# lyeemax/IS-VINS

Hardware: AMD Instinct MI355X
Metric: sliding-window solves/sec (11 KF, ~300 landmarks) (higher is better)
Workload: dtype f64; 1 GPU; 1024 independent synthetic sliding windows per GPU (N=11 KF, Nvo=5, L=300 landmarks, F~1070 reprojection factors each; BASELINE config 4 batch of config-2 windows), full backendOptimization(): NUM_ITERATIONS=10 dogleg iterations + update() + double2vector + MargForward/MargBackward on every window; windows_per_gpu=1024, windows_total=1024, frames=11, landmarks=300, factors_total=1095427

## Files before the change

is-vins_amd/csrc/isv_backend.hip:

```cpp
#include <hip/hip_runtime.h>
#include <atomic>
#include <chrono>
#include <cstdio>
#include <cstdlib>
#include <cstring>
#include <string>
#include <thread>
#include <sched.h>
#include <vector>
#include <algorithm>
#include "isv_device_types.h"
#include "isv_kernels.h"

#include "isv_batch_buffers.h"

extern "C" int isv_abi_version(void) { return ISV_ABI_VERSION; }

extern "C" const char *isv_backend_last_error(const isv_backend_t *h) { return h ? h->err.c_str() : "null handle"; }

extern "C" void isv_backend_destroy(isv_backend_t *h) {
    if (!h) return;
    (void)hipSetDevice(h->device);
    if (h->graph_exec) (void)hipGraphExecDestroy(h->graph_exec);
    if (h->seq && h->seq_free) h->seq_free(h->seq);
// ... 531 lines not shown
        for (int i = 0; i < ISV_MAX_TRACE; i++) out[3] += act[i];
    }
    return ISV_OK;
}

static uint64_t fnv1a(const void *p, size_t n) { uint64_t x = 1469598103934665603ull; for (size_t i = 0; i < n; i++) { x ^= ((const unsigned char *)p)[i]; x *= 1099511628211ull; } return x; }

extern "C" int isv_batch_optimize(isv_backend_t *h, int32_t sync) {
    if (!h || !h->resident) return ISV_ERR_INVALID_ARG;
    ENTER(h);
    DevBatch &d = h->d; hipStream_t st = h->stream;
    memset(h->last_counts, 0, sizeof(h->last_counts));
    const bool profile = (sync & 2) != 0 && !h->prof_ev.empty();
    static const bool use_graph = getenv("ISV_GRAPH") != nullptr;
    if (use_graph && !profile) {
        d.sw_global = 0; d.ctl_stage_lm = 0; d.dg_stage_ph = 0;
        const uint64_t key = fnv1a(&d, sizeof(d));
        HIPCHK(h, hipEventRecord(h->ev[0], st));
        if (!h->graph_exec || h->graph_key != key) {
            if (h->graph_exec) { (void)hipGraphExecDestroy(h->graph_exec); h->graph_exec = nullptr; }
            hipGraph_t g = nullptr;
            HIPCHK(h, hipStreamBeginCapture(st, hipStreamCaptureModeThreadLocal));
            int rcg = ISV_OK;
            if (hipMemsetAsync(d.act, 0, sizeof(int32_t) * ISV_MAX_TRACE, st) != hipSuccess) rcg = ISV_ERR_DEVICE;
            if (rcg == ISV_OK) rcg = restore_initial(h);
            if (rcg == ISV_OK) {
                hipLaunchKernelGGL(k_vector2double, dim3(d.B), dim3(64), 0, st, d);
                rcg = isv_solver_enqueue(h->d, h->hc, st, h->stream2, h->fj, h->last_counts, nullptr, h->err);
            }
            const hipError_t ec = hipStreamEndCapture(st, &g);
            if (rcg != ISV_OK || ec != hipSuccess) { if (g) (void)hipGraphDestroy(g); h->err = "hipGraph capture failed"; return rcg != ISV_OK ? rcg : ISV_ERR_DEVICE; }
// ... 249 lines not shown
```

is-vins_amd/csrc/isv_build_solve_sb.hip:

```cpp
#include <hip/hip_runtime.h>
#include "isv_kernels.h"
#include "isv_device_math.h"
#include "isv_chain.h"
#include "isv_lin_gram.h"
#include "isv_rank1.h"
#include "isv_dogleg.h"

#ifdef ISV_STAMP
#define STAMP(k) do { if (t == 0) { unsigned long long now_ = wall_clock64(); d.dbg[(size_t)w * 64 + (k) + (MODE == 1 ? 32 : 0)] += (double)(now_ - t_last); t_last = now_; } } while (0)
#else
#define STAMP(k) do {} while (0)
#endif
#define LS 512
__host__ __device__ inline int sb_nred(int N, int prior_H_sz) {
    int m = LS;
    if (prior_H_sz > m) m = prior_H_sz;
    if (36 * N > m) m = 36 * N;
    if (30 * N > m) m = 30 * N;
    return (m + 1) & ~1;
}
#define RCH 32

DEV int sbt(int I, int J, int N) { return (I == J ? I : N + J) * 36; }

// ... 1037 lines not shown
            __syncthreads();
            if ((int)threadIdx.x >= 64 * nwaves) return;
            rank1_body<NT, TPW, 64, 1, EX>(d);
        }
    }
    else build_solve_sb_body<BIG, NC, 1>(d, lds);
}
template <bool BIG, int NC, bool EX>
__global__ __launch_bounds__(LS, 2) void k_pose_dogleg(DevBatch d) {
    extern __shared__ __align__(16) double lds[];
    __shared__ double red[256];
    __shared__ int s_accept;
    build_solve_sb_body<BIG, NC, 2>(d, lds);
    __syncthreads();
    if (threadIdx.x >= 256) return;
    dogleg_body<EX>(d, blockIdx.x, threadIdx.x, red);
    __syncthreads();
    step_control_body<true, EX>(d, blockIdx.x, threadIdx.x, lds, red, s_accept);
}
template __global__ void k_pose_dogleg<false, 11, false>(DevBatch);
template __global__ void k_pose_dogleg<false, 0, false>(DevBatch);
template __global__ void k_pose_dogleg<false, 0, true>(DevBatch);
template __global__ void k_lin_gram_chain<false, false, 0, 0>(DevBatch);
template __global__ void k_lin_gram_chain<false, false, 11, 0>(DevBatch);
template __global__ void k_lin_gram_chain<false, true, 0, 0>(DevBatch);
template __global__ void k_lin_gram_chain<true, false, 0, 0>(DevBatch);
template __global__ void k_lin_gram_chain<true, true, 0, 0>(DevBatch);
template __global__ void k_lin_gram_chain<false, true, 0, 7>(DevBatch);
template __global__ void k_build_solve_sb<false, 0, 0>(DevBatch);
template __global__ void k_build_solve_sb<false, 11, 0>(DevBatch);
template __global__ void k_build_solve_sb<true, 0, 0>(DevBatch);
template __global__ void k_build_solve_sb<false, 0, 1>(DevBatch);
template __global__ void k_build_solve_sb<false, 11, 1>(DevBatch);
// ... 18 lines not shown
```

is-vins_amd/csrc/isv_device_types.h:

```cpp
#pragma once
#include <stdint.h>
#include "../../include/isvins_backend.h"

#define ISV_TILE 64
#define ISV_MAX_FRAMES 32
#define ISV_MARG_WS 1408
#define ISV_SPLIT_MAX_GROUPS 32
#ifndef ISV_SPLIT_MIN_PASSES
#define ISV_SPLIT_MIN_PASSES 4
#endif
#define ISV_FUSED_MAX_FACTORS 8192
#define ISV_IMU_IN 64
#define IMU_DP 0
#define IMU_DQ 3
#define IMU_DV 7
#define IMU_LBA 10
#define IMU_LBG 13
#define IMU_DT 16
#define IMU_DP_DBA 17
#define IMU_DP_DBG 26
#define IMU_DQ_DBG 35
#define IMU_DV_DBA 44
#define IMU_DV_DBG 53

// ... 82 lines not shown
    double *st_ws;
    int32_t split_cap, _pad4;
    double *cs_ws;
    double *r1_part;
    double *Tvis;
    int32_t force_retry, init_mode;
    int32_t prior_H_sz, tvis_sz, wd_ld, max_lm;
    int32_t marg_scratch_sz, lds_T;
    int32_t force_invalid, _pad2;
    double min_radius;
    int32_t *pg_rec;
    double *pg_pts;
    int32_t *pg_wstart;
    double *flm;
    int32_t fused_visual;
    int32_t bs_split, _pad3;
    int32_t ctl_stage_lm, dg_stage_ph;
    int32_t lg_lcap;
    int32_t Nr, est_ex;
    double *Wex;
    double *flmx;
    double *ex_part;
    double *strip_ex;
};
```

is-vins_amd/csrc/isv_dogleg.h:

```cpp
#pragma once
#include <hip/hip_runtime.h>
#include "isv_kernels.h"
#include "isv_device_math.h"
#include "isv_proj_factor.h"
#include "isv_prior_factor.h"
#include "isv_imu_factor.h"

template <int K>
DEV void block_sums(double (&v)[K], double *red , int t) {
#pragma unroll
    for (int k = 0; k < K; k++) {
#pragma unroll
        for (int off = 32; off > 0; off >>= 1) v[k] += __shfl_down(v[k], off, 64);
    }
    if ((t & 63) == 0) {
#pragma unroll
        for (int k = 0; k < K; k++) red[(t >> 6) * K + k] = v[k];
    }
    __syncthreads();
#pragma unroll
    for (int k = 0; k < K; k++) v[k] = ((red[k] + red[K + k]) + red[2 * K + k]) + red[3 * K + k];
    __syncthreads();
}

#ifdef ISV_STAMP
#define DSTAMP(k) do { if (t == (k >= 56 ? 64 : 0)) { unsigned long long now_ = wall_clock64(); d.dbg[(size_t)w * 64 + (k)] += (double)(now_ - (k >= 56 ? t1_last : t_last)); if (k >= 56) t1_last = now_; else t_last = now_; } } while (0)
#else
#define DSTAMP(k) do {} while (0)
#endif
template <bool EX>
DEV void backsub_landmark(const DevBatch &d, const int l, const int fw0, const double *zs, const double *us, const double mu) {
            const unsigned m0 = d.lm_meta[l];
            const int h = (int)(m0 & 255), k = (int)((m0 >> 8) & 255);
            const double *wv = d.W + (size_t)(fw0 + (int)(m0 >> 16) + l) * 6;
            const double sl = d.scale_l[l], E = d.lmE[l], gl = d.lmG[l], Dl = d.diag_l[l];
            double wz = 0, wu = 0;
            for (int o = 0; o < k; o += 2) {
                const int o1 = o + 1 < k ? o + 1 : o;
                const double2 a01 = *reinterpret_cast<const double2 *>(wv + 6 * o), a23 = *reinterpret_cast<const double2 *>(wv + 6 * o + 2),
                              a45 = *reinterpret_cast<const double2 *>(wv + 6 * o + 4);
                const double2 b01 = *reinterpret_cast<const double2 *>(wv + 6 * o1), b23 = *reinterpret_cast<const double2 *>(wv + 6 * o1 + 2),
                              b45 = *reinterpret_cast<const double2 *>(wv + 6 * o1 + 4);
                const double *z = zs + 15 * (h + o), *u = us + 15 * (h + o);
                wz += a01.x * z[0] + a01.y * z[1] + a23.x * z[2] + a23.y * z[3] + a45.x * z[4] + a45.y * z[5];
                wu += a01.x * u[0] + a01.y * u[1] + a23.x * u[2] + a23.y * u[3] + a45.x * u[4] + a45.y * u[5];
                if (o + 1 < k) {
                    const double *z1 = zs + 15 * (h + o + 1), *u1 = us + 15 * (h + o + 1);
                    wz += b01.x * z1[0] + b01.y * z1[1] + b23.x * z1[2] + b23.y * z1[3] + b45.x * z1[4] + b45.y * z1[5];
                    wu += b01.x * u1[0] + b01.y * u1[1] + b23.x * u1[2] + b23.y * u1[3] + b45.x * u1[4] + b45.y * u1[5];
                }
            }
            if (EX) {
                const double *we = d.Wex + (size_t)l * 6, *z = zs + 15 * d.Nr, *u = us + 15 * d.Nr;
                for (int c6 = 0; c6 < 6; c6++) { wz += we[c6] * z[c6]; wu += we[c6] * u[c6]; }
            }
            const double Es = sl * sl * E, Dl2 = Dl * Dl;
            const double yl = (sl * gl - sl * wz) / (Es + mu * Dl2);
            d.gn_l[l] = -Dl * yl;
            const double ul = sl * sl * gl / Dl2, cl = sl * sl / (Es + mu * Dl2);
            d.lm_aterm[l] = cl * wu * wu + 2.0 * ul * wu + E * ul * ul;
}

template <bool EX>
DEV void dogleg_body(DevBatch &d, const int w, const int t, double *red) {
    SolveState &st = d.st[w];
    if (st.termination != ISV_TERM_RUNNING) return;
    const int n = d.np, N = d.N, l0 = d.lm_off[w], l1 = d.lm_off[w + 1];
    const double *gp = d.grad_p + (size_t)w * n, *gnp = d.gn_p + (size_t)w * n;
    const double *Dp = d.diag_p + (size_t)w * n, *scp = d.scale_p + (size_t)w * n;
    double *dp = d.delta_p + (size_t)w * n;
    if (st.ls_fail) {
        if (t == 0) { st.step_valid = 0; st.iteration += 1; st.fresh = 0; }
        return;
    }
#ifdef ISV_STAMP
    unsigned long long t_last = wall_clock64(), t1_last = t_last;
#endif
    if (d.lds_T) {
        extern __shared__ __align__(16) double dynp[];
        double *const sPr = dynp + (size_t)(N - 1) * 48 + (size_t)d.n_prior_slots * 16;
        prior_stage_records(d, w, sPr + (size_t)d.n_prior_slots * 20, t, 256);
        double *const sPHw = sPr + prior_lds_bytes(d.n_prior_slots, false) / sizeof(double) + 992 + n;
// ... 3 lines not shown
#pragma unroll
            for (int u = 0; u < 4; u++) { const int i = i0 + 256 * u; v4[u] = PHg[i < d.prior_H_sz ? i : d.prior_H_sz - 1]; }
#pragma unroll
            for (int u = 0; u < 4; u++) { const int i = i0 + 256 * u; if (i < d.prior_H_sz) sPHw[i] = v4[u]; }
        }
    }
    double a = 0, b = 0, c = 0, e = 0;
    for (int i = t; i < n; i += 256) { a += gp[i] * gp[i]; b += gnp[i] * gnp[i]; c += gp[i] * gnp[i]; }
    if (st.fresh && !d.bs_split) {
        extern __shared__ __align__(16) double dyn0[];
        double *zs = dyn0, *us = dyn0 + n;
        for (int i = t; i < n; i += 256) { zs[i] = d.zp[(size_t)w * n + i]; us[i] = d.up[(size_t)w * n + i]; }
        __syncthreads();
        const double mu = st.mu;
        const int fw0 = d.f_off[w];
        for (int l = l0 + t; l < l1; l += 256) backsub_landmark<EX>(d, l, fw0, zs, us, mu);
    }
    for (int lq = l0 + t; lq < l1; lq += 4 * 256) {
        double gl4[4], nl4[4], at4[4];
#pragma unroll
        for (int u = 0; u < 4; u++) { const int l = lq + 256 * u < l1 ? lq + 256 * u : l1 - 1; gl4[u] = d.grad_l[l]; nl4[u] = d.gn_l[l]; at4[u] = d.lm_aterm[l]; }
#pragma unroll
        for (int u = 0; u < 4; u++) if (lq + 256 * u < l1) { a += gl4[u] * gl4[u]; b += nl4[u] * nl4[u]; c += gl4[u] * nl4[u]; e += at4[u]; }
    }
    DSTAMP(48);
    double sums4[4] = {a, b, c, e};
    block_sums<4>(sums4, red, t);
    const double g2 = sums4[0], gn2 = sums4[1], gdotgn = sums4[2], aterm = sums4[3];
    double alpha = st.alpha;
    if (st.fresh) alpha = g2 / (st.qT + aterm);
    const double radius = st.radius, gn_norm = sqrt(gn2), g_norm = sqrt(g2);
    double cg, cn, step_norm_scaled;
// ... 1 lines not shown
    if (gn_norm <= radius) { cg = 0; cn = 1; step_norm_scaled = gn_norm; }
    else if (g_norm * alpha >= radius) { cg = -(radius / g_norm); cn = 0; step_norm_scaled = radius; }
    else {
        const double b_dot_a = -alpha * gdotgn;
        const double a_sq = pow(alpha * g_norm, 2.0);
        const double bma_sq = a_sq - 2 * b_dot_a + pow(gn_norm, 2.0);
        const double cc = b_dot_a - a_sq;
        const double dd = sqrt(cc * cc + bma_sq * (pow(radius, 2.0) - a_sq));
        const double beta = (cc <= 0) ? (dd - cc) / bma_sq : (radius * radius - a_sq) / (dd + cc);
        cg = -alpha * (1.0 - beta); cn = beta; step_norm_scaled = 0; need_norm = true;
    }
    double sn = 0;
    for (int i = t; i < n; i += 256) {
        const double s = cg * gp[i] + cn * gnp[i];
        sn += s * s;
        dp[i] = s / Dp[i] * scp[i];
    }
    for (int lq = l0 + t; lq < l1; lq += 4 * 256) {
        double gl4[4], nl4[4], dg4[4], sc4[4], lam4[4];
#pragma unroll
        for (int u = 0; u < 4; u++) { const int l = lq + 256 * u < l1 ? lq + 256 * u : l1 - 1; gl4[u] = d.grad_l[l]; nl4[u] = d.gn_l[l]; dg4[u] = d.diag_l[l]; sc4[u] = d.scale_l[l]; lam4[u] = d.lam[l]; }
#pragma unroll
        for (int u = 0; u < 4; u++) if (lq + 256 * u < l1) {
            const int l = lq + 256 * u;
            const double s = cg * gl4[u] + cn * nl4[u];
            sn += s * s;
            const double dl = s / dg4[u] * sc4[u];
            d.delta_l[l] = dl;
            d.clam[l] = lam4[u] + dl;
        }
    }
    double sums1[1] = {sn};
    block_sums<1>(sums1, red, t);
    const double sn_tot = sums1[0];
    if (need_norm) step_norm_scaled = sqrt(sn_tot);
    __syncthreads();
    double dn = 0, xn = 0;
    for (int i = t; i < N; i += 256) {
        const double *x = d.pose + ((size_t)w * N + i) * 7, *sb = d.sb + ((size_t)w * N + i) * 9;
        double *xc = d.cpose + ((size_t)w * N + i) * 7, *sc = d.csb + ((size_t)w * N + i) * 9;
        double xp[7];
        pose_plus(x, dp + 15 * i, xp);
        for (int k = 0; k < 7; k++) { xc[k] = xp[k]; const double df = x[k] - xp[k]; dn += df * df; xn += x[k] * x[k]; }
        for (int k = 0; k < 9; k++) { const double v = sb[k] + dp[15 * i + 6 + k]; sc[k] = v; const double df = sb[k] - v; dn += df * df; xn += sb[k] * sb[k]; }
    }
    for (int lq = l0 + t; lq < l1; lq += 4 * 256) {
        double lam4[4], cl4[4];
#pragma unroll
        for (int u = 0; u < 4; u++) { const int l = lq + 256 * u < l1 ? lq + 256 * u : l1 - 1; lam4[u] = d.lam[l]; cl4[u] = d.clam[l]; }
#pragma unroll
        for (int u = 0; u < 4; u++) if (lq + 256 * u < l1) { const double df = lam4[u] - cl4[u]; dn += df * df; xn += lam4[u] * lam4[u]; }
    }
    DSTAMP(49);
    double sums2[2] = {dn, xn};
    block_sums<2>(sums2, red, t);
    const double dn_tot = sums2[0], xn_tot = sums2[1];
    if (t == 0) {
        st.alpha = alpha; st.dogleg_step_norm = step_norm_scaled;
        st.step_norm = sqrt(dn_tot); st.x_norm = sqrt(xn_tot);
        st.step_valid = 1; st.iteration += 1; st.fresh = 0;
    }
    if (!d.lds_T) return;
    extern __shared__ __align__(16) double dyn[];
    const int NIw = N - 1, slots = d.n_prior_slots;
    double *sImu = dyn;
    double *sMod = sImu + NIw * 16;
    double *sPm = sMod + NIw * 32;
    double *sPrior = sPm + (size_t)slots * 16;
    {
        double *sDpw = sPrior + prior_lds_bytes(slots, false) / sizeof(double) + 992;
        for (int i = t; i < n; i += 256) sDpw[i] = dp[i];
    }
    __syncthreads();
    DSTAMP(50);
#ifdef ISV_STAMP
    t1_last = wall_clock64();
#endif
    const int lane = t & 63, wv = t >> 6;
    double *const sRaw = sPrior, *const sW = sPrior + (size_t)slots * 10;
    const PriorRecs PR = prior_recs_at(d, sPrior + (size_t)slots * 20);
    const int n_rp = d.n_rp[w];
    double *const sHb = sPrior + prior_lds_bytes(slots, false) / sizeof(double);
    const double *sDp = sHb + 992;
    if (wv == 0) {
        if (lane < NIw) {
            const size_t f = (size_t)w * NIw + lane;
            if (!d.imu_skip[f]) {
                const double *pi = d.cpose + ((size_t)w * N + lane) * 7, *si = d.csb + ((size_t)w * N + lane) * 9;
// ... 53 lines not shown
                double s = 0;
#pragma unroll
                for (int b = 0; b < 30; b++) s += sH[a >= b ? a * (a + 1) / 2 + b : b * (b + 1) / 2 + a] * dd[b];
                sMod[q * 32 + a] = dd[a] * (sH[465 + a] + 0.5 * s);
            }
        }
    }
    DSTAMP(51);
    DSTAMP(56);
#ifdef ISV_STAMP
    if (t == 128) d.dbg[(size_t)w * 64 + 62] += (double)(wall_clock64() - t1_last);
#endif
    __syncthreads();
    DSTAMP(52);
    double *sR2 = sHb;
    if (wv == 3) prior_residual_costs(d, PR, w, n_rp, sRaw, sW, d.prior_cost_c, lane);
    for (int tq = t; tq < NIw * 15; tq += 256) {
        const int q = tq / 15, row = tq - 15 * q;
        const size_t f = (size_t)w * NIw + q;
        const double *S = d.imu_sqrt + f * 225 + row * 15;
        double r = 0;
#pragma unroll
        for (int k = 0; k < 15; k++) r += S[k] * sImu[q * 16 + k];
        sR2[tq] = r * r;
    }
    __syncthreads();
    if (t < NIw) {
        const size_t f = (size_t)w * NIw + t;
        double c2 = 0, m = 0;
        if (!d.imu_skip[f]) {
            for (int k = 0; k < 15; k++) c2 += sR2[t * 15 + k];
            for (int a = 0; a < 30; a++) m += sMod[t * 32 + a];
        }
        d.imu_cost_c[f] = 0.5 * c2;
        d.imu_model[f] = m;
    } else if (t >= 64 && t < 64 + slots) {
        const int q = t - 64;
        double m = 0;
        for (int a = 0; a < 12; a++) m += sPm[q * 16 + a];
        d.prior_model[(size_t)w * slots + q] = m;
    }
    DSTAMP(53);
}
template <bool FUSED, bool EX> DEV void step_control_body(DevBatch &d, const int w, const int t, double *cl, double *red, int &s_accept);

template <bool FUSED, bool EX>
DEV void step_control_body(DevBatch &d, const int w, const int t, double *cl, double *red, int &s_accept) {
    SolveState &st = d.st[w];
    if (st.termination != ISV_TERM_RUNNING) return;
    const int N = d.N;
    double S = 0, M = 0;
    if (st.step_valid) {
        double s = 0, m = 0;
        if (FUSED) {
            double *sC = cl, *sEx = cl + N * 12, *sX = sEx + 12, *sD = sX + N * 12, *sL = sD + N * 6;
            const int l0w = d.lm_off[w], Lww = d.lm_off[w + 1] - l0w;
            const bool stage = d.ctl_stage_lm != 0;
            if (stage) {
                for (int e = t; e < Lww; e += 256) {
                    const double *pp = d.lm_pts_i + (size_t)(l0w + e) * 3;
                    sL[6 * e] = pp[0]; sL[6 * e + 1] = pp[1]; sL[6 * e + 2] = pp[2];
                    sL[6 * e + 3] = d.clam[l0w + e]; sL[6 * e + 4] = d.lam[l0w + e]; sL[6 * e + 5] = d.delta_l[l0w + e];
                }
            }
            if (t < N) {
                const double *p = d.cpose + ((size_t)w * N + t) * 7;
                double R[9]; q_to_R(q_from_pose(p), R);
#pragma unroll
                for (int k = 0; k < 9; k++) sC[t * 12 + k] = R[k];
                sC[t * 12 + 9] = p[0]; sC[t * 12 + 10] = p[1]; sC[t * 12 + 11] = p[2];
            } else if (t >= 64 && t < 64 + N) {
                const int fr = t - 64;
                const double *p = d.pose + ((size_t)w * N + fr) * 7;
                double R[9]; q_to_R(q_from_pose(p), R);
#pragma unroll
                for (int k = 0; k < 9; k++) sX[fr * 12 + k] = R[k];
                sX[fr * 12 + 9] = p[0]; sX[fr * 12 + 10] = p[1]; sX[fr * 12 + 11] = p[2];
                const double *dp = d.delta_p + (size_t)w * d.np + 15 * fr;
#pragma unroll
                for (int k = 0; k < 6; k++) sD[fr * 6 + k] = dp[k];
            } else if (t == 128) {
                const double *e = d.ex + (size_t)w * 7;
                double R[9]; q_to_R(q_from_pose(e), R);
#pragma unroll
                for (int k = 0; k < 9; k++) sEx[k] = R[k];
                sEx[9] = e[0]; sEx[10] = e[1]; sEx[11] = e[2];
            }
            __syncthreads();
            const double *exC = EX ? sC + d.Nr * 12 : sEx, *exX = EX ? sX + d.Nr * 12 : sEx;
            double ric[9], tic[3];
#pragma unroll
            for (int k = 0; k < 9; k++) ric[k] = exC[k];
#pragma unroll
// ... 39 lines not shown
                proj_residual_dir(Ri, Pi, Rj, Pj, ric, tic, d.proj_sqrt_info, lam_l, pi3[0], pi3[1], pi3[2], pj.x, pj.y,
                                  sD + fi * 6, sD + fj * 6, dl_l, rx0, rx1, m0, m1);
                const double rp = 1.0 / (1.0 + (rx0 * rx0 + rx1 * rx1));
                m += rp * (m0 * (rx0 + m0 / 2.0) + m1 * (rx1 + m1 / 2.0));
            }
        } else {
            const int f_end = d.f_off[w + 1];
            for (int f0 = d.f_off[w] + t; f0 < f_end; f0 += 8 * 256) {
                double cs[8], ms[8];
#pragma unroll
                for (int u = 0; u < 8; u++) { const int f = f0 + 256 * u < f_end ? f0 + 256 * u : f_end - 1; cs[u] = d.fcost_c[f]; ms[u] = d.fmodel[f]; }
#pragma unroll
                for (int u = 0; u < 8; u++) if (f0 + 256 * u < f_end) { s += cs[u]; m += ms[u]; }
            }
        }
        for (int i = t; i < N - 1; i += 256) { s += d.imu_cost_c[(size_t)w * (N - 1) + i]; m += d.imu_model[(size_t)w * (N - 1) + i]; }
        for (int i = t; i < d.n_prior_slots; i += 256) { s += d.prior_cost_c[(size_t)w * d.n_prior_slots + i]; m += d.prior_model[(size_t)w * d.n_prior_slots + i]; }
        double sm[2] = {s, m};
        block_sums<2>(sm, red, t);
        S = sm[0]; M = sm[1];
    }
    if (t == 0) {
        s_accept = 0;
        const int it = st.iteration;
        double *tc = d.trace_cost + (size_t)w * ISV_MAX_TRACE, *tr = d.trace_radius + (size_t)w * ISV_MAX_TRACE;
        double *ts = d.trace_step + (size_t)w * ISV_MAX_TRACE; int32_t *ta = d.trace_acc + (size_t)w * ISV_MAX_TRACE;
        const double model_cost_change = -M;
        const bool valid = st.step_valid && (model_cost_change > 0.0) && !(it <= d.force_invalid);
        d.cost_c[w] = S; d.model[w] = M;
        if (!valid) {
            st.invalid += 1;
            if (st.invalid >= 5) st.termination = st.ls_fail ? ISV_TERM_LINEAR_SOLVER : ISV_TERM_INVALID_STEPS;
// ... 21 lines not shown
                    tc[it] = cand_cost; tr[it] = st.radius; ts[it] = step_norm; ta[it] = 1;
                } else {
                    st.radius *= 0.5; st.reuse = 1;
                    tc[it] = cand_cost; tr[it] = st.radius; ts[it] = step_norm; ta[it] = 0;
                }
                if (it >= d.max_iter) st.termination = ISV_TERM_MAX_ITERATIONS;
                else if (st.radius <= d.min_radius) st.termination = ISV_TERM_MIN_RADIUS;
            }
        }
    }
    __syncthreads();
    if (s_accept) {
        const int l0 = d.lm_off[w], l1 = d.lm_off[w + 1];
        for (int i = t; i < N * 7; i += 256) d.pose[(size_t)w * N * 7 + i] = d.cpose[(size_t)w * N * 7 + i];
        for (int i = t; i < N * 9; i += 256) d.sb[(size_t)w * N * 9 + i] = d.csb[(size_t)w * N * 9 + i];
        for (int l = l0 + t; l < l1; l += 256) d.lam[l] = d.clam[l];
    }
}
```

is-vins_amd/csrc/isv_prior_factor.h:

```cpp
#pragma once
#include "isv_device_types.h"
#include "isv_device_math.h"

#define PRL_RAW 82
#define PRL_W 90
#define PRL_S 82
DEV void relpose_jac(const double *dt, const double *dR, const double *pi, const double *pj, double *res, double *Ji, double *Jj) {
    Quat Qi = q_from_pose(pi), Qj = q_from_pose(pj);
    double Ri[9], Rj[9], dd[3], qd[3], M1[9], M2[9], lg[3], Jr[9], S[9], nJ[9], T1[9], T2[9];
    q_to_R(Qi, Ri); q_to_R(Qj, Rj);
    for (int k = 0; k < 3; k++) dd[k] = pj[k] - pi[k];
    q_rot(q_inv(Qi), dd, qd);
    m3_mul_nt(dR, Rj, M1); m3_mul(M1, Ri, M2);
    so3_log(q_from_R(M2), lg);
    for (int k = 0; k < 3; k++) { res[k] = dt[k] - qd[k]; res[3 + k] = lg[k]; }
    so3_rjac_inv(lg, Jr); skew3(qd, S);
    for (int k = 0; k < 36; k++) { Ji[k] = 0; Jj[k] = 0; }
    for (int k = 0; k < 9; k++) nJ[k] = -Jr[k];
    m3_mul_nt(nJ, Ri, T1); m3_mul(T1, Rj, T2);
    for (int a = 0; a < 3; a++) for (int b = 0; b < 3; b++) {
        Ji[a * 6 + b] = Ri[b * 3 + a]; Ji[a * 6 + 3 + b] = -S[a * 3 + b]; Ji[(3 + a) * 6 + 3 + b] = Jr[a * 3 + b];
        Jj[a * 6 + b] = -Ri[b * 3 + a]; Jj[(3 + a) * 6 + 3 + b] = T2[a * 3 + b];
    }
}
// ... 192 lines not shown
            q_rot(so3_mul(Rm, q_conj(Rq)), nZ, v);
            raw[0] = v[0]; raw[1] = v[1];
            if (JAC) {
                double S[9], Rmm[9], Bm[9];
                skew3(v, S); q_to_R(Rm, Rmm); m3_mul(S, Rmm, Bm);
#pragma unroll
                for (int k = 0; k < 12; k++) rawJ[k] = 0;
#pragma unroll
                for (int a = 0; a < 2; a++)
#pragma unroll
                    for (int b = 0; b < 3; b++) rawJ[a * 6 + 3 + b] = Bm[a * 3 + b];
            }
        }
    }
}
DEV void prior_residual_costs(const DevBatch &d, const PriorRecs &R, int w, int n_rp, const double *sRaw, double *sW, double *cost_out, int t) {
    constexpr int RAWS = 10, WS = 10;
    const int slots = d.n_prior_slots;
    for (int e = t; e < slots * 9; e += 64) {
        const int s = e / 9, row = e - 9 * s;
        const PriorDesc p = prior_desc(d, R, s, n_rp);
        const int dim = p.kind == 1 ? 9 : (p.kind == 3 ? 2 : 6);
        if (!p.valid || row >= dim) continue;
        const double *raw = sRaw + s * RAWS;
        double v = 0;
        for (int k = 0; k < dim; k++) v += p.S[row * dim + k] * raw[k];
        sW[s * WS + row] = v;
    }
    ISV_WSYNC();
    for (int s = t; s < slots; s += 64) {
        const PriorDesc p = prior_desc(d, R, s, n_rp);
        const int dim = p.kind == 1 ? 9 : (p.kind == 3 ? 2 : 6);
        double cost = 0.0;
        if (p.valid) {
            const double *wr = sW + s * WS;
            double ssum = 0;
            for (int k = 0; k < dim; k++) ssum += wr[k] * wr[k];
            cost = 0.5 * log(1.0 + ssum);
        }
        cost_out[(size_t)w * slots + s] = cost;
    }
}

template <bool JAC, bool WAVE>
DEV void prior_linearize_body(const DevBatch &d, const double *pose_src, const double *sb_src, double *cost_out, int gate, int w, double *lds, int s0 = 0, int sstride = 1) {
    const int t = WAVE ? (int)(threadIdx.x & 63) : (int)threadIdx.x;
    const int slots = d.n_prior_slots;
    if (gate) {
        const SolveState &ss = d.st[w];
        if (!(ss.termination == ISV_TERM_RUNNING && (gate == 1 ? ss.need_linearize != 0 : ss.step_valid != 0))) return;
    }
    const int n_rp = d.n_rp[w];
    constexpr int RAWS = JAC ? PRL_RAW : 10, WS = JAC ? PRL_W : 10;
    double *sRaw = lds, *sW = lds + (size_t)slots * RAWS, *sRec = sW + (size_t)slots * WS;
    double *strip = d.prior_strip + (size_t)w * d.prior_strip_sz;
// ... 44 lines not shown
```

is-vins_amd/csrc/isv_solver.hip:

```cpp
#include <hip/hip_runtime.h>
#include <cstring>
#include <cstdio>
#include <cstdlib>
#include <map>
#include <mutex>
#include "isv_kernels.h"
#include "isv_device_math.h"
#include "isv_proj_factor.h"
#include "isv_prior_factor.h"
#include "isv_imu_factor.h"
#include "isv_batch_buffers.h"

extern size_t build_solve_lds_bytes(int N);
template <bool BIG, int NC, int MODE> __global__ void k_build_solve_sb(DevBatch d);
extern size_t build_solve_sb_bytes(int N, int prior_H_sz);
extern size_t build_solve_cs_doubles(int N);
template <bool EX, bool BIG, int NC, int NT> __global__ void k_lin_gram_chain(DevBatch d);
__global__ void k_front(DevBatch d);
template <bool BIG, int NC, bool EX> __global__ void k_pose_dogleg(DevBatch d);
extern size_t front_lds_bytes(int N, int slots);
template <bool BIG, int NC> __global__ void k_build_solve_st(DevBatch d);
extern size_t build_solve_st_bytes(int N, int prior_H_sz);
extern size_t build_solve_st_ws_doubles(int N);
__global__ void k_model_imu_prior(DevBatch d);
// ... 21 lines not shown
        d.trace_cost[(size_t)w * ISV_MAX_TRACE + k] = 0; d.trace_radius[(size_t)w * ISV_MAX_TRACE + k] = 0;
        d.trace_step[(size_t)w * ISV_MAX_TRACE + k] = 0; d.trace_acc[(size_t)w * ISV_MAX_TRACE + k] = 0;
    }
}

#include "isv_dogleg.h"

template <bool CONTROL, bool EX>
__global__ __launch_bounds__(256, 4) void k_dogleg(DevBatch d) {
    __shared__ double red[256];
    __shared__ int s_accept;
    const int w = blockIdx.x, t = threadIdx.x;
#ifdef ISV_STAMP
    const unsigned long long tk0 = wall_clock64();
#endif
    dogleg_body<EX>(d, w, t, red);
#ifdef ISV_STAMP
    const unsigned long long tk1 = wall_clock64();
#endif
    if (CONTROL) {
        extern __shared__ __align__(16) double dync[];
        __syncthreads();
        step_control_body<true, EX>(d, w, t, dync, red, s_accept);
    }
#ifdef ISV_STAMP
    if (t == 0) { d.dbg[(size_t)w * 64 + 54] += (double)(tk1 - tk0); d.dbg[(size_t)w * 64 + 55] += (double)(wall_clock64() - tk1); }
#endif
}
template __global__ void k_dogleg<false, false>(DevBatch);
template __global__ void k_dogleg<true, false>(DevBatch);
template __global__ void k_dogleg<false, true>(DevBatch);
template __global__ void k_dogleg<true, true>(DevBatch);

__global__ __launch_bounds__(128) void k_backsub_split(DevBatch d) {
    extern __shared__ __align__(16) double zsus[];
    const int w = blockIdx.x, t = threadIdx.x;
    const SolveState &st = d.st[w];
    if (st.termination != ISV_TERM_RUNNING || st.ls_fail || !st.fresh) return;
    const int n = d.np, l0 = d.lm_off[w], l1 = d.lm_off[w + 1];
    const int l = l0 + (int)blockIdx.y * 128 + t;
    if (l0 + (int)blockIdx.y * 128 >= l1) return;
    double *zs = zsus, *us = zsus + n;
    for (int i = t; i < n; i += 128) { zs[i] = d.zp[(size_t)w * n + i]; us[i] = d.up[(size_t)w * n + i]; }
    __syncthreads();
    if (l < l1) backsub_landmark<false>(d, l, d.f_off[w], zs, us, st.mu);
}


template <bool FUSED, bool EX>
__global__ __launch_bounds__(256) void k_step_control(DevBatch d) {
    extern __shared__ __align__(16) double cl[];
    __shared__ double red[256];
    __shared__ int s_accept;
    step_control_body<FUSED, EX>(d, blockIdx.x, threadIdx.x, cl, red, s_accept);
}

__global__ __launch_bounds__(64) void k_finalize(DevBatch d, int do_update) {
    const int w = blockIdx.x, lane = threadIdx.x;
    if (ISV_SEQ_IDLE(d, w)) return;
    const int N = d.N, v = d.Nvo - 1;
    const double *pose = d.pose + (size_t)w * N * 7, *sb = d.sb + (size_t)w * N * 9;
    double *Ps = d.Ps + (size_t)w * N * 3, *Rs = d.Rs + (size_t)w * N * 9, *Vs = d.Vs + (size_t)w * N * 3;
    double *Bas = d.Bas + (size_t)w * N * 3, *Bgs = d.Bgs + (size_t)w * N * 3;
    double origin_R0[3], origin_P0[3], origin_R00[3], R00[9], rot_diff[9], Rs0[9];
    for (int k = 0; k < 9; k++) Rs0[k] = Rs[k];
    R2ypr(Rs0, origin_R0);
    for (int k = 0; k < 3; k++) origin_P0[k] = Ps[k];
    q_to_R(q_from_pose(pose), R00);
    R2ypr(R00, origin_R00);
// ... 91 lines not shown
    *p = (T *)q;
    return ISV_OK;
}
#define TRYA(x) do { int rc_ = (x); if (rc_ != ISV_OK) return rc_; } while (0)
hipError_t isv_raise_dynamic_lds(const void *fn, int device, size_t lds) {
    static std::mutex mtx;
    static std::map<std::pair<const void *, int>, size_t> raised;
    std::lock_guard<std::mutex> lk(mtx);
    size_t &cur = raised[{fn, device}];
    if (lds <= cur) return hipSuccess;
    const hipError_t e = hipFuncSetAttribute(fn, hipFuncAttributeMaxDynamicSharedMemorySize, (int)lds);
    if (e == hipSuccess) cur = lds;
    return e;
}
static size_t dogleg_lds_bytes(const DevBatch &d) {
    return (d.lds_T ? ((size_t)(d.N - 1) * 48 + (size_t)d.n_prior_slots * 16 + 992 + (size_t)d.np + (d.dg_stage_ph ? (size_t)d.prior_H_sz : 0)) * sizeof(double) + prior_lds_bytes(d.n_prior_slots, false) : 0) + 2 * (size_t)d.np * sizeof(double);
}
static size_t step_control_lds_bytes(const DevBatch &d) { return ((size_t)30 * d.N + 12 + (d.ctl_stage_lm ? 6 * (size_t)d.lg_lcap : 0)) * sizeof(double); }
#define ISV_CTL_STAGE_MAX_BYTES ((size_t)36 * 1024)

template <int MODE> static const void *solve_sb_kernel(int N, bool generic_n) {
    if (N == 11 && !generic_n) return (const void *)k_build_solve_sb<false, 11, MODE>;
    return N <= 11 ? (const void *)k_build_solve_sb<false, 0, MODE> : (const void *)k_build_solve_sb<true, 0, MODE>;
}
template <int NT> static void set_rank1_kernels(SolverKernel *k, bool ex, bool split, size_t lds_r1, size_t lds_sp) {
    constexpr int TPW = NT <= 5 ? 1 : NT <= 7 ? 2 : 3;
    constexpr unsigned threads = 64 * ((NT * (NT + 1) / 2 + TPW - 1) / TPW);
    k[KR_RANK1] = {ex ? (const void *)k_rank1_mfma<NT, TPW, 64, 1, true> : (const void *)k_rank1_mfma<NT, TPW, 64, 1, false>, threads, lds_r1};
    if (split) {
        k[KR_RANK1_SPLIT] = {(const void *)k_rank1_split<NT, TPW>, threads, lds_r1};
        k[KR_SCHUR_SPLIT] = {(const void *)k_schur_split<NT, TPW>, threads, lds_sp};
    }
}
// ... 121 lines not shown
}

template <typename... A> static void launch(const SolverKernel &k, dim3 grid, size_t lds, hipStream_t s, A... a) {
    void *args[] = {&a...};
    (void)hipLaunchKernel(k.fn, grid, dim3(k.threads), args, lds, s);
}

int isv_solver_enqueue(DevBatch &d, const SolverHost &hc, hipStream_t st, hipStream_t st2, hipEvent_t *fj, int64_t *counts, hipEvent_t *prof_ev, std::string &err) {
#define PROF(slot, fam, which) do { if (prof_ev) (void)hipEventRecord(prof_ev[((slot) * ISV_PROF_FAMILIES + (fam)) * 2 + (which)], st); } while (0)
    const SolverKernel *K = hc.kern;
    const size_t NI = (size_t)d.B * (d.N - 1);
    const size_t lds_proj = 4 * proj_lds_doubles_per_wave(d.N, 0) * sizeof(double), lds_proj1 = 4 * proj_lds_doubles_per_wave(d.N, 1) * sizeof(double);
    if (hc.one_stream) st2 = st;
    d.ctl_stage_lm = (6 * (size_t)d.lg_lcap * sizeof(double) <= ISV_CTL_STAGE_MAX_BYTES) ? 1 : 0;
    d.dg_stage_ph = 1;
    if (ISV_LDS_PER_CU / ((dogleg_lds_bytes(d) > step_control_lds_bytes(d) ? dogleg_lds_bytes(d) : step_control_lds_bytes(d)) + 2304) * (size_t)hc.n_cus < (size_t)d.B) d.dg_stage_ph = 0;
    const size_t lds_dg = dogleg_lds_bytes(d), lds_sc = step_control_lds_bytes(d);
    const size_t lds_dgc = lds_dg > lds_sc ? lds_dg : lds_sc;
    const size_t dg_by_lds = ISV_LDS_PER_CU / (lds_dgc + 2304);
    const size_t res_dogleg_ctl = (size_t)hc.n_cus * ((size_t)hc.dogleg_per_cu_regs < dg_by_lds ? (size_t)hc.dogleg_per_cu_regs : dg_by_lds);
    const bool control_in_wg = d.lds_T && ((size_t)d.Ftot <= (size_t)4096 * d.B || d.est_ex);
    const bool fuse_control = control_in_wg && !hc.split_control && (size_t)d.B <= res_dogleg_ctl;
    const int n_cus = hc.n_cus;
    const bool cs = hc.chain_split;
    const bool fused = d.lds_T && d.fused_visual;
    d.sw_global = (d.sw_part && hc.sw_global_ok && (d.B > 256 || hc.debug_sw_global)) ? 1 : 0;
    const int lgw = (fused && d.B <= n_cus && !hc.lg_batch_waves && lin_gram_lds_bytes(d.Nr, !d.sw_global, d.est_ex != 0, LG_WAVES_SMALL, d.lg_lcap) <= ISV_LDS_PER_CU) ? LG_WAVES_SMALL : LG_WAVES;
    const bool lg_chain = cs && fused && lgw == LG_WAVES_SMALL;
    const int Pmax = (d.lg_lcap + 63) / 64, PmaxH = (d.max_lm + 63) / 64, GrMax = PmaxH < d.split_cap ? PmaxH : d.split_cap;
    const bool split = d.lds_T && d.r1_part && !hc.no_split && Pmax >= ISV_SPLIT_MIN_PASSES && d.split_cap >= 2;
    const bool r1_in_lg = lg_chain && K[KR_LIN_GRAM_CHAIN_R1].fn && !split;
    const bool bsub_split = split && d.lg_lcap > 1024;
    d.bs_split = bsub_split ? 1 : 0;
// ... 168 lines not shown
```

Measured before the change: 194,900 windows/s.

## Hand off dogleg landmark and cost data to step control through LDS

```diff
diff --git a/is-vins_amd/csrc/isv_backend.hip b/is-vins_amd/csrc/isv_backend.hip
--- a/is-vins_amd/csrc/isv_backend.hip
+++ b/is-vins_amd/csrc/isv_backend.hip
@@ -569,7 +569,7 @@
     const bool profile = (sync & 2) != 0 && !h->prof_ev.empty();
     static const bool use_graph = getenv("ISV_GRAPH") != nullptr;
     if (use_graph && !profile) {
-        d.sw_global = 0; d.ctl_stage_lm = 0; d.dg_stage_ph = 0;
+        d.sw_global = 0; d.ctl_stage_lm = 0; d.dg_stage_ph = 0; d.dg_hand_lm = 0;
         const uint64_t key = fnv1a(&d, sizeof(d));
         HIPCHK(h, hipEventRecord(h->ev[0], st));
         if (!h->graph_exec || h->graph_key != key) {
diff --git a/is-vins_amd/csrc/isv_build_solve_sb.hip b/is-vins_amd/csrc/isv_build_solve_sb.hip
--- a/is-vins_amd/csrc/isv_build_solve_sb.hip
+++ b/is-vins_amd/csrc/isv_build_solve_sb.hip
@@ -1075,9 +1075,10 @@
     build_solve_sb_body<BIG, NC, 2>(d, lds);
     __syncthreads();
     if (threadIdx.x >= 256) return;
-    dogleg_body<EX>(d, blockIdx.x, threadIdx.x, red);
+    double *const hand = lds + dogleg_hand_off(d);
+    dogleg_body<EX>(d, blockIdx.x, threadIdx.x, red, hand);
     __syncthreads();
-    step_control_body<true, EX>(d, blockIdx.x, threadIdx.x, lds, red, s_accept);
+    step_control_body<true, EX>(d, blockIdx.x, threadIdx.x, lds, red, s_accept, hand);
 }
 template __global__ void k_pose_dogleg<false, 11, false>(DevBatch);
 template __global__ void k_pose_dogleg<false, 0, false>(DevBatch);
diff --git a/is-vins_amd/csrc/isv_device_types.h b/is-vins_amd/csrc/isv_device_types.h
--- a/is-vins_amd/csrc/isv_device_types.h
+++ b/is-vins_amd/csrc/isv_device_types.h
@@ -120,7 +120,7 @@
     int32_t *pg_wstart;
     double *flm;
     int32_t fused_visual;
-    int32_t bs_split, _pad3;
+    int32_t bs_split, dg_hand_lm;
     int32_t ctl_stage_lm, dg_stage_ph;
     int32_t lg_lcap;
     int32_t Nr, est_ex;
diff --git a/is-vins_amd/csrc/isv_dogleg.h b/is-vins_amd/csrc/isv_dogleg.h
--- a/is-vins_amd/csrc/isv_dogleg.h
+++ b/is-vins_amd/csrc/isv_dogleg.h
@@ -29,11 +29,13 @@
 #define DSTAMP(k) do {} while (0)
 #endif
 template <bool EX>
-DEV void backsub_landmark(const DevBatch &d, const int l, const int fw0, const double *zs, const double *us, const double mu) {
+DEV void backsub_landmark(const DevBatch &d, const int l, const int fw0, const double *zs, const double *us, const double mu,
+                          double &gn, double &at, double &Dl, double &sl) {
             const unsigned m0 = d.lm_meta[l];
             const int h = (int)(m0 & 255), k = (int)((m0 >> 8) & 255);
             const double *wv = d.W + (size_t)(fw0 + (int)(m0 >> 16) + l) * 6;
-            const double sl = d.scale_l[l], E = d.lmE[l], gl = d.lmG[l], Dl = d.diag_l[l];
+            const double E = d.lmE[l], gl = d.lmG[l];
+            sl = d.scale_l[l]; Dl = d.diag_l[l];
             double wz = 0, wu = 0;
             for (int o = 0; o < k; o += 2) {
                 const int o1 = o + 1 < k ? o + 1 : o;
@@ -56,16 +58,61 @@
             }
             const double Es = sl * sl * E, Dl2 = Dl * Dl;
             const double yl = (sl * gl - sl * wz) / (Es + mu * Dl2);
-            d.gn_l[l] = -Dl * yl;
+            gn = -Dl * yl;
+            d.gn_l[l] = gn;
             const double ul = sl * sl * gl / Dl2, cl = sl * sl / (Es + mu * Dl2);
-            d.lm_aterm[l] = cl * wu * wu + 2.0 * ul * wu + E * ul * ul;
+            at = cl * wu * wu + 2.0 * ul * wu + E * ul * ul;
+            d.lm_aterm[l] = at;
+}
+template <bool EX>
+DEV void backsub_landmark(const DevBatch &d, const int l, const int fw0, const double *zs, const double *us, const double mu) {
+    double gn, at, Dl, sl;
+    backsub_landmark<EX>(d, l, fw0, zs, us, mu, gn, at, Dl, sl);
+}
+
+__host__ __device__ static inline size_t dogleg_dp_off(const DevBatch &d) {
+    return (size_t)(d.N - 1) * 48 + (size_t)d.n_prior_slots * 16 + prior_lds_bytes(d.n_prior_slots, false) / sizeof(double) + 992;
+}
+__host__ __device__ static inline size_t dogleg_eval_doubles(const DevBatch &d) { return dogleg_dp_off(d) + (size_t)d.np + (d.dg_stage_ph ? (size_t)d.prior_H_sz : 0); }
+__host__ __device__ static inline size_t step_control_doubles(const DevBatch &d) { return (size_t)30 * d.N + 12 + (d.ctl_stage_lm ? 6 * (size_t)d.lg_lcap : 0); }
+__host__ __device__ static inline size_t dogleg_hand_off(const DevBatch &d) {
+    const size_t a = dogleg_eval_doubles(d), b = step_control_doubles(d);
+    return a > b ? a : b;
+}
+__host__ __device__ static inline size_t dogleg_hand_doubles(const DevBatch &d) {
+    return 2 * (size_t)(d.N - 1) + 2 * (size_t)d.n_prior_slots + (d.dg_hand_lm ? 3 * (size_t)d.lg_lcap : 0);
+}
+
+template <class LD>
+DEV void dogleg_landmark_step(const DevBatch &d, const int l0, const int l1, const int t, const double cg, const double cn, double &sn, double *hL, LD ld) {
+    for (int lq = l0 + t; lq < l1; lq += 4 * 256) {
+        double gl4[4], nl4[4], dg4[4], sc4[4], lam4[4];
+#pragma unroll
+        for (int u = 0; u < 4; u++) { const int l = lq + 256 * u < l1 ? lq + 256 * u : l1 - 1; ld(l, gl4[u], nl4[u], dg4[u], sc4[u], lam4[u]); }
+#pragma unroll
+        for (int u = 0; u < 4; u++) if (lq + 256 * u < l1) {
+            const int l = lq + 256 * u;
+            const double s = cg * gl4[u] + cn * nl4[u];
+            sn += s * s;
+            const double dl = s / dg4[u] * sc4[u];
+            d.delta_l[l] = dl;
+            const double cl = lam4[u] + dl;
+            d.clam[l] = cl;
+            if (hL) { const int e3 = 3 * (l - l0); hL[e3] = cl; hL[e3 + 1] = lam4[u]; hL[e3 + 2] = dl; }
+        }
+    }
 }
 
 template <bool EX>
-DEV void dogleg_body(DevBatch &d, const int w, const int t, double *red) {
+DEV void dogleg_body(DevBatch &d, const int w, const int t, double *red, double *hand) {
     SolveState &st = d.st[w];
     if (st.termination != ISV_TERM_RUNNING) return;
     const int n = d.np, N = d.N, l0 = d.lm_off[w], l1 = d.lm_off[w + 1];
+    double *const hL = (hand && d.dg_hand_lm) ? hand + 2 * (N - 1) + 2 * d.n_prior_slots : nullptr;
+    extern __shared__ __align__(16) double dynd[];
+    double *const sDpw = d.lds_T ? dynd + dogleg_dp_off(d) : nullptr;
+    const bool chip = hL && st.fresh && !d.bs_split && 2 * (l1 - l0) <= 992;
+    double *const sT = chip ? sDpw - 992 : nullptr;
     const double *gp = d.grad_p + (size_t)w * n, *gnp = d.gn_p + (size_t)w * n;
     const double *Dp = d.diag_p + (size_t)w * n, *scp = d.scale_p + (size_t)w * n;
     double *dp = d.delta_p + (size_t)w * n;
@@ -99,8 +146,20 @@
         __syncthreads();
         const double mu = st.mu;
         const int fw0 = d.f_off[w];
+        if (chip) {
+            for (int l = l0 + t; l < l1; l += 256) {
+                const int e3 = 3 * (l - l0), e2 = 2 * (l - l0);
+                const double gr = d.grad_l[l], lm = d.lam[l];
+                double gn, at, Dl, sl;
+                backsub_landmark<EX>(d, l, fw0, zs, us, mu, gn, at, Dl, sl);
+                asm("" : "+v"(gn)); asm("" : "+v"(at));
+                a += gr * gr; b += gn * gn; c += gr * gn; e += at;
+                hL[e3] = gn; hL[e3 + 1] = lm; hL[e3 + 2] = gr; sT[e2] = Dl; sT[e2 + 1] = sl;
+            }
+        } else
         for (int l = l0 + t; l < l1; l += 256) backsub_landmark<EX>(d, l, fw0, zs, us, mu);
     }
+    if (!chip)
     for (int lq = l0 + t; lq < l1; lq += 4 * 256) {
         double gl4[4], nl4[4], at4[4];
 #pragma unroll
@@ -132,36 +191,35 @@
     for (int i = t; i < n; i += 256) {
         const double s = cg * gp[i] + cn * gnp[i];
         sn += s * s;
-        dp[i] = s / Dp[i] * scp[i];
-    }
-    for (int lq = l0 + t; lq < l1; lq += 4 * 256) {
-        double gl4[4], nl4[4], dg4[4], sc4[4], lam4[4];
-#pragma unroll
-        for (int u = 0; u < 4; u++) { const int l = lq + 256 * u < l1 ? lq + 256 * u : l1 - 1; gl4[u] = d.grad_l[l]; nl4[u] = d.gn_l[l]; dg4[u] = d.diag_l[l]; sc4[u] = d.scale_l[l]; lam4[u] = d.lam[l]; }
-#pragma unroll
-        for (int u = 0; u < 4; u++) if (lq + 256 * u < l1) {
-            const int l = lq + 256 * u;
-            const double s = cg * gl4[u] + cn * nl4[u];
-            sn += s * s;
-            const double dl = s / dg4[u] * sc4[u];
-            d.delta_l[l] = dl;
-            d.clam[l] = lam4[u] + dl;
-        }
-    }
-    double sums1[1] = {sn};
-    block_sums<1>(sums1, red, t);
-    const double sn_tot = sums1[0];
-    if (need_norm) step_norm_scaled = sqrt(sn_tot);
+        const double v = s / Dp[i] * scp[i];
+        dp[i] = v;
+        if (sDpw) sDpw[i] = v;
+    }
+    if (chip) dogleg_landmark_step(d, l0, l1, t, cg, cn, sn, hL, [&](int l, double &gl, double &nl, double &dg, double &sc, double &lam) {
+        const int e3 = 3 * (l - l0), e2 = 2 * (l - l0);
+        gl = hL[e3 + 2]; nl = hL[e3]; dg = sT[e2]; sc = sT[e2 + 1]; lam = hL[e3 + 1];
+    });
+    else dogleg_landmark_step(d, l0, l1, t, cg, cn, sn, hL, [&](int l, double &gl, double &nl, double &dg, double &sc, double &lam) {
+        gl = d.grad_l[l]; nl = d.gn_l[l]; dg = d.diag_l[l]; sc = d.scale_l[l]; lam = d.lam[l];
+    });
     __syncthreads();
+    const double *dpr = sDpw ? sDpw : dp;
     double dn = 0, xn = 0;
     for (int i = t; i < N; i += 256) {
         const double *x = d.pose + ((size_t)w * N + i) * 7, *sb = d.sb + ((size_t)w * N + i) * 9;
         double *xc = d.cpose + ((size_t)w * N + i) * 7, *sc = d.csb + ((size_t)w * N + i) * 9;
         double xp[7];
-        pose_plus(x, dp + 15 * i, xp);
+        pose_plus(x, dpr + 15 * i, xp);
         for (int k = 0; k < 7; k++) { xc[k] = xp[k]; const double df = x[k] - xp[k]; dn += df * df; xn += x[k] * x[k]; }
-        for (int k = 0; k < 9; k++) { const double v = sb[k] + dp[15 * i + 6 + k]; sc[k] = v; const double df = sb[k] - v; dn += df * df; xn += sb[k] * sb[k]; }
-    }
+        for (int k = 0; k < 9; k++) { const double v = sb[k] + dpr[15 * i + 6 + k]; sc[k] = v; const double df = sb[k] - v; dn += df * df; xn += sb[k] * sb[k]; }
+    }
+    if (hL) {
+        for (int l = l0 + t; l < l1; l += 256) {
+            const int e3 = 3 * (l - l0);
+            const double lm = hL[e3 + 1], df = lm - hL[e3];
+            dn += df * df; xn += lm * lm;
+        }
+    } else
     for (int lq = l0 + t; lq < l1; lq += 4 * 256) {
         double lam4[4], cl4[4];
 #pragma unroll
@@ -170,9 +228,10 @@
         for (int u = 0; u < 4; u++) if (lq + 256 * u < l1) { const double df = lam4[u] - cl4[u]; dn += df * df; xn += lam4[u] * lam4[u]; }
     }
     DSTAMP(49);
-    double sums2[2] = {dn, xn};
-    block_sums<2>(sums2, red, t);
-    const double dn_tot = sums2[0], xn_tot = sums2[1];
+    double sums3[3] = {sn, dn, xn};
+    block_sums<3>(sums3, red, t);
+    if (need_norm) step_norm_scaled = sqrt(sums3[0]);
+    const double dn_tot = sums3[1], xn_tot = sums3[2];
     if (t == 0) {
         st.alpha = alpha; st.dogleg_step_norm = step_norm_scaled;
         st.step_norm = sqrt(dn_tot); st.x_norm = sqrt(xn_tot);
@@ -185,11 +244,6 @@
     double *sMod = sImu + NIw * 16;
     double *sPm = sMod + NIw * 32;
     double *sPrior = sPm + (size_t)slots * 16;
-    {
-        double *sDpw = sPrior + prior_lds_bytes(slots, false) / sizeof(double) + 992;
-        for (int i = t; i < n; i += 256) sDpw[i] = dp[i];
-    }
-    __syncthreads();
     DSTAMP(50);
 #ifdef ISV_STAMP
     t1_last = wall_clock64();
@@ -273,7 +327,7 @@
     __syncthreads();
     DSTAMP(52);
     double *sR2 = sHb;
-    if (wv == 3) prior_residual_costs(d, PR, w, n_rp, sRaw, sW, d.prior_cost_c, lane);
+    if (wv == 3) prior_residual_costs(d, PR, w, n_rp, sRaw, sW, d.prior_cost_c, lane, hand ? hand + 2 * NIw : nullptr);
     for (int tq = t; tq < NIw * 15; tq += 256) {
         const int q = tq / 15, row = tq - 15 * q;
         const size_t f = (size_t)w * NIw + q;
@@ -291,35 +345,42 @@
             for (int k = 0; k < 15; k++) c2 += sR2[t * 15 + k];
             for (int a = 0; a < 30; a++) m += sMod[t * 32 + a];
         }
-        d.imu_cost_c[f] = 0.5 * c2;
+        const double ic = 0.5 * c2;
+        d.imu_cost_c[f] = ic;
         d.imu_model[f] = m;
+        if (hand) { hand[t] = ic; hand[NIw + t] = m; }
     } else if (t >= 64 && t < 64 + slots) {
         const int q = t - 64;
         double m = 0;
         for (int a = 0; a < 12; a++) m += sPm[q * 16 + a];
         d.prior_model[(size_t)w * slots + q] = m;
+        if (hand) hand[2 * NIw + slots + q] = m;
     }
     DSTAMP(53);
 }
-template <bool FUSED, bool EX> DEV void step_control_body(DevBatch &d, const int w, const int t, double *cl, double *red, int &s_accept);
+template <bool FUSED, bool EX> DEV void step_control_body(DevBatch &d, const int w, const int t, double *cl, double *red, int &s_accept, const double *hand);
 
 template <bool FUSED, bool EX>
-DEV void step_control_body(DevBatch &d, const int w, const int t, double *cl, double *red, int &s_accept) {
+DEV void step_control_body(DevBatch &d, const int w, const int t, double *cl, double *red, int &s_accept, const double *hand) {
     SolveState &st = d.st[w];
     if (st.termination != ISV_TERM_RUNNING) return;
     const int N = d.N;
+    const bool stage = FUSED && d.ctl_stage_lm != 0;
+    double *const sL = cl + N * 30 + 12;
     double S = 0, M = 0;
     if (st.step_valid) {
         double s = 0, m = 0;
         if (FUSED) {
-            double *sC = cl, *sEx = cl + N * 12, *sX = sEx + 12, *sD = sX + N * 12, *sL = sD + N * 6;
+            double *sC = cl, *sEx = cl + N * 12, *sX = sEx + 12, *sD = sX + N * 12;
             const int l0w = d.lm_off[w], Lww = d.lm_off[w + 1] - l0w;
-            const bool stage = d.ctl_stage_lm != 0;
+            const double *const hL = (hand && d.dg_hand_lm) ? hand + 2 * (N - 1) + 2 * d.n_prior_slots : nullptr;
+            const double *const hDp = (hand && step_control_doubles(d) <= dogleg_dp_off(d)) ? cl + dogleg_dp_off(d) : nullptr;
             if (stage) {
                 for (int e = t; e < Lww; e += 256) {
                     const double *pp = d.lm_pts_i + (size_t)(l0w + e) * 3;
                     sL[6 * e] = pp[0]; sL[6 * e + 1] = pp[1]; sL[6 * e + 2] = pp[2];
-                    sL[6 * e + 3] = d.clam[l0w + e]; sL[6 * e + 4] = d.lam[l0w + e]; sL[6 * e + 5] = d.delta_l[l0w + e];
+                    if (hL) { sL[6 * e + 3] = hL[3 * e]; sL[6 * e + 4] = hL[3 * e + 1]; sL[6 * e + 5] = hL[3 * e + 2]; }
+                    else { sL[6 * e + 3] = d.clam[l0w + e]; sL[6 * e + 4] = d.lam[l0w + e]; sL[6 * e + 5] = d.delta_l[l0w + e]; }
                 }
             }
             if (t < N) {
@@ -335,7 +396,7 @@
 #pragma unroll
                 for (int k = 0; k < 9; k++) sX[fr * 12 + k] = R[k];
                 sX[fr * 12 + 9] = p[0]; sX[fr * 12 + 10] = p[1]; sX[fr * 12 + 11] = p[2];
-                const double *dp = d.delta_p + (size_t)w * d.np + 15 * fr;
+                const double *dp = hDp ? hDp + 15 * fr : d.delta_p + (size_t)w * d.np + 15 * fr;
 #pragma unroll
                 for (int k = 0; k < 6; k++) sD[fr * 6 + k] = dp[k];
             } else if (t == 128) {
@@ -405,8 +466,14 @@
                 for (int u = 0; u < 8; u++) if (f0 + 256 * u < f_end) { s += cs[u]; m += ms[u]; }
             }
         }
+        if (FUSED && hand) {
+            const double *hP = hand + 2 * (N - 1);
+            if (t < N - 1) { s += hand[t]; m += hand[N - 1 + t]; }
+            if (t < d.n_prior_slots) { s += hP[t]; m += hP[d.n_prior_slots + t]; }
+        } else {
         for (int i = t; i < N - 1; i += 256) { s += d.imu_cost_c[(size_t)w * (N - 1) + i]; m += d.imu_model[(size_t)w * (N - 1) + i]; }
         for (int i = t; i < d.n_prior_slots; i += 256) { s += d.prior_cost_c[(size_t)w * d.n_prior_slots + i]; m += d.prior_model[(size_t)w * d.n_prior_slots + i]; }
+        }
         double sm[2] = {s, m};
         block_sums<2>(sm, red, t);
         S = sm[0]; M = sm[1];
@@ -458,6 +525,7 @@
         const int l0 = d.lm_off[w], l1 = d.lm_off[w + 1];
         for (int i = t; i < N * 7; i += 256) d.pose[(size_t)w * N * 7 + i] = d.cpose[(size_t)w * N * 7 + i];
         for (int i = t; i < N * 9; i += 256) d.sb[(size_t)w * N * 9 + i] = d.csb[(size_t)w * N * 9 + i];
-        for (int l = l0 + t; l < l1; l += 256) d.lam[l] = d.clam[l];
-    }
-}
+        if (stage) { for (int l = l0 + t; l < l1; l += 256) d.lam[l] = sL[6 * (l - l0) + 3]; }
+        else for (int l = l0 + t; l < l1; l += 256) d.lam[l] = d.clam[l];
+    }
+}
diff --git a/is-vins_amd/csrc/isv_prior_factor.h b/is-vins_amd/csrc/isv_prior_factor.h
--- a/is-vins_amd/csrc/isv_prior_factor.h
+++ b/is-vins_amd/csrc/isv_prior_factor.h
@@ -230,7 +230,7 @@
         }
     }
 }
-DEV void prior_residual_costs(const DevBatch &d, const PriorRecs &R, int w, int n_rp, const double *sRaw, double *sW, double *cost_out, int t) {
+DEV void prior_residual_costs(const DevBatch &d, const PriorRecs &R, int w, int n_rp, const double *sRaw, double *sW, double *cost_out, int t, double *cost_lds = nullptr) {
     constexpr int RAWS = 10, WS = 10;
     const int slots = d.n_prior_slots;
     for (int e = t; e < slots * 9; e += 64) {
@@ -255,6 +255,7 @@
             cost = 0.5 * log(1.0 + ssum);
         }
         cost_out[(size_t)w * slots + s] = cost;
+        if (cost_lds) cost_lds[s] = cost;
     }
 }
 
diff --git a/is-vins_amd/csrc/isv_solver.hip b/is-vins_amd/csrc/isv_solver.hip
--- a/is-vins_amd/csrc/isv_solver.hip
+++ b/is-vins_amd/csrc/isv_solver.hip
@@ -59,14 +59,15 @@
 #ifdef ISV_STAMP
     const unsigned long long tk0 = wall_clock64();
 #endif
-    dogleg_body<EX>(d, w, t, red);
+    extern __shared__ __align__(16) double dync[];
+    double *const hand = CONTROL ? dync + dogleg_hand_off(d) : nullptr;
+    dogleg_body<EX>(d, w, t, red, hand);
 #ifdef ISV_STAMP
     const unsigned long long tk1 = wall_clock64();
 #endif
     if (CONTROL) {
-        extern __shared__ __align__(16) double dync[];
         __syncthreads();
-        step_control_body<true, EX>(d, w, t, dync, red, s_accept);
+        step_control_body<true, EX>(d, w, t, dync, red, s_accept, hand);
     }
 #ifdef ISV_STAMP
     if (t == 0) { d.dbg[(size_t)w * 64 + 54] += (double)(tk1 - tk0); d.dbg[(size_t)w * 64 + 55] += (double)(wall_clock64() - tk1); }
@@ -97,7 +98,7 @@
     extern __shared__ __align__(16) double cl[];
     __shared__ double red[256];
     __shared__ int s_accept;
-    step_control_body<FUSED, EX>(d, blockIdx.x, threadIdx.x, cl, red, s_accept);
+    step_control_body<FUSED, EX>(d, blockIdx.x, threadIdx.x, cl, red, s_accept, nullptr);
 }
 
 __global__ __launch_bounds__(64) void k_finalize(DevBatch d, int do_update) {
@@ -219,9 +220,10 @@
     return e;
 }
 static size_t dogleg_lds_bytes(const DevBatch &d) {
-    return (d.lds_T ? ((size_t)(d.N - 1) * 48 + (size_t)d.n_prior_slots * 16 + 992 + (size_t)d.np + (d.dg_stage_ph ? (size_t)d.prior_H_sz : 0)) * sizeof(double) + prior_lds_bytes(d.n_prior_slots, false) : 0) + 2 * (size_t)d.np * sizeof(double);
-}
-static size_t step_control_lds_bytes(const DevBatch &d) { return ((size_t)30 * d.N + 12 + (d.ctl_stage_lm ? 6 * (size_t)d.lg_lcap : 0)) * sizeof(double); }
+    return (d.lds_T ? dogleg_eval_doubles(d) * sizeof(double) : 0) + 2 * (size_t)d.np * sizeof(double);
+}
+static size_t step_control_lds_bytes(const DevBatch &d) { return step_control_doubles(d) * sizeof(double); }
+static size_t dogleg_control_lds_bytes(const DevBatch &d) { return (dogleg_hand_off(d) + dogleg_hand_doubles(d)) * sizeof(double); }
 #define ISV_CTL_STAGE_MAX_BYTES ((size_t)36 * 1024)
 
 template <int MODE> static const void *solve_sb_kernel(int N, bool generic_n) {
@@ -373,9 +375,12 @@
     if (hc.one_stream) st2 = st;
     d.ctl_stage_lm = (6 * (size_t)d.lg_lcap * sizeof(double) <= ISV_CTL_STAGE_MAX_BYTES) ? 1 : 0;
     d.dg_stage_ph = 1;
-    if (ISV_LDS_PER_CU / ((dogleg_lds_bytes(d) > step_control_lds_bytes(d) ? dogleg_lds_bytes(d) : step_control_lds_bytes(d)) + 2304) * (size_t)hc.n_cus < (size_t)d.B) d.dg_stage_ph = 0;
+    d.dg_hand_lm = (d.lds_T && d.ctl_stage_lm) ? 1 : 0;
+    if (d.dg_hand_lm && dogleg_control_lds_bytes(d) > (size_t)64 * 1024) d.dg_hand_lm = 0;
+    auto dgc_bytes = [&]() { const size_t a = dogleg_lds_bytes(d), b = step_control_lds_bytes(d), c = d.lds_T ? dogleg_control_lds_bytes(d) : 0; return a > b ? (a > c ? a : c) : (b > c ? b : c); };
+    if (ISV_LDS_PER_CU / (dgc_bytes() + 2304) * (size_t)hc.n_cus < (size_t)d.B) d.dg_stage_ph = 0;
     const size_t lds_dg = dogleg_lds_bytes(d), lds_sc = step_control_lds_bytes(d);
-    const size_t lds_dgc = lds_dg > lds_sc ? lds_dg : lds_sc;
+    const size_t lds_dgc = dgc_bytes();
     const size_t dg_by_lds = ISV_LDS_PER_CU / (lds_dgc + 2304);
     const size_t res_dogleg_ctl = (size_t)hc.n_cus * ((size_t)hc.dogleg_per_cu_regs < dg_by_lds ? (size_t)hc.dogleg_per_cu_regs : dg_by_lds);
     const bool control_in_wg = d.lds_T && ((size_t)d.Ftot <= (size_t)4096 * d.B || d.est_ex);
```

New measurement: 196,600 windows/s, median of 6. No clear change (+0.9%).
